# achiever04/face-recognition-platform

Hardware: AMD Instinct MI355X
Metric: faces/sec (detect+embed+match) on 1080p @ 100k gallery (higher is better)
Workload: dtype f16; 1 GPU; 32x1080x1920 BGR frames per GPU per step resident in HBM, host results out every step, 2 batches in flight per GPU (one handle = one stream each, used round-robin), forced K=10 faces/frame, 100000-identity fp16 gallery, FRPDet detector fp16 + ArcFace IResNet-100 fp16 (synthetic seeded weights); batch_frames=32, faces_per_frame=10, gallery=100000, streams=1, lanes=2, lane_warmup_steps=20

## Files before the change

face-recognition-platform_amd/csrc/decode_nms.hip:

```cpp
#include <hip/hip_runtime.h>
#include <stdint.h>
#include "frp_internal.h"

namespace frp {

#define NMS_CAP 1024
#define NT 1024

__device__ __forceinline__ unsigned sortable16(unsigned short h) {
    if ((h & 0x7fffu) > 0x7c00u) return 0u;
    return (h & 0x8000u) ? (unsigned)(unsigned short)(~h) : (unsigned)(h | 0x8000u);
}
__device__ __forceinline__ bool is_candidate(_Float16 lg, float lt) {
    return lt == -INFINITY ? true : (float)lg >= lt;
}

struct FrameView {
    const _Float16 *h0, *h1, *h2;
    int w0, w1, w2;
    int e0, e1;
};

__device__ __forceinline__ const _Float16* anchor_ptr(const FrameView& fv, int idx, int& level, int& x, int& y) {
    level = idx < fv.e0 ? 0 : (idx < fv.e1 ? 1 : 2);
    const int li = idx - (level == 0 ? 0 : (level == 1 ? fv.e0 : fv.e1));
    const int wl = level == 0 ? fv.w0 : (level == 1 ? fv.w1 : fv.w2);
    const _Float16* base = level == 0 ? fv.h0 : (level == 1 ? fv.h1 : fv.h2);
    const int pos = li >> 1, a = li & 1;
    y = pos / wl;
    x = pos - y * wl;
    return base + (long)pos * 32 + a * 15;
}

__device__ __forceinline__ FrameView frame_view(const DecodeParams& p, int b, int& A) {
    FrameView fv;
    fv.h0 = p.head[0] + (long)b * p.hl[0] * p.wl[0] * 32;
    fv.h1 = p.head[1] + (long)b * p.hl[1] * p.wl[1] * 32;
    fv.h2 = p.head[2] + (long)b * p.hl[2] * p.wl[2] * 32;
    fv.w0 = p.wl[0]; fv.w1 = p.wl[1]; fv.w2 = p.wl[2];
    fv.e0 = p.hl[0] * p.wl[0] * 2;
    fv.e1 = fv.e0 + p.hl[1] * p.wl[1] * 2;
    A = fv.e1 + p.hl[2] * p.wl[2] * 2;
    return fv;
}

__global__ __launch_bounds__(256) void gather_logits_kernel(DecodeParams p) {
    int A;
    const FrameView fv = frame_view(p, blockIdx.y, A);
    const int i = blockIdx.x * 256 + threadIdx.x;
    if (i >= A) return;
    int lv, x, y;
    p.logits[(long)blockIdx.y * A + i] = anchor_ptr(fv, i, lv, x, y)[0];
}

__global__ __launch_bounds__(NT) void decode_nms_kernel(DecodeParams p) {
    __shared__ unsigned long long keys[NMS_CAP];
    __shared__ int hist[4096];
    __shared__ float bx1[NMS_CAP], by1[NMS_CAP], bx2[NMS_CAP], by2[NMS_CAP], barea[NMS_CAP];
    __shared__ unsigned char supp[NMS_CAP];
    __shared__ int s_cnt, s_digit, s_need, s_keepn;
    __shared__ int s_keep[FRP_MAX_FACES_CAP];
    __shared__ int wsum[NT / 64];

    const int b = blockIdx.x;
    const int tid = threadIdx.x;
    int A;
    const FrameView fv = frame_view(p, b, A);
    const float lt = p.logit_thresh;

    if (tid == 0) { s_cnt = 0; s_keepn = 0; }
    __syncthreads();
    const _Float16* dense = p.logits + (long)b * A;
    int local = 0;
    for (int i = tid; i < A; i += NT) local += is_candidate(dense[i], lt) ? 1 : 0;
#pragma unroll
    for (int o = 32; o > 0; o >>= 1) local += __shfl_xor(local, o);
    if ((tid & 63) == 0) atomicAdd(&s_cnt, local);
    __syncthreads();
    const int total = s_cnt;
    __syncthreads();

    unsigned long long T = 0ull;
    if (total > NMS_CAP) {
        unsigned long long prefix = 0ull;
        int need = NMS_CAP;
        for (int pass = 0; pass < 3; ++pass) {
            const int shift = 24 - 12 * pass;
            for (int i = tid; i < 4096; i += NT) hist[i] = 0;
            __syncthreads();
            for (int i = tid; i < A; i += NT) {
                const _Float16 lg = dense[i];
                if (is_candidate(lg, lt)) {
                    const unsigned long long k = ((unsigned long long)sortable16(__builtin_bit_cast(unsigned short, lg)) << 20) |
                                                 (unsigned long long)(0xFFFFF - i);
                    if (pass == 0 || (k >> (shift + 12)) == prefix) atomicAdd(&hist[(int)((k >> shift) & 0xFFF)], 1);
                }
            }
            __syncthreads();
            const int b0 = tid * 4;
            const int h0 = hist[b0], h1 = hist[b0 + 1], h2 = hist[b0 + 2], h3 = hist[b0 + 3];
            const int mine = h0 + h1 + h2 + h3;
            int v = mine;
#pragma unroll
            for (int o = 1; o < 64; o <<= 1) {
                const int n = __shfl_down(v, o);
                if ((tid & 63) + o < 64) v += n;
            }
            if ((tid & 63) == 0) wsum[tid >> 6] = v;
            __syncthreads();
            int above_waves = 0;
            for (int w = (tid >> 6) + 1; w < NT / 64; ++w) above_waves += wsum[w];
            const int suffix_incl = v + above_waves;
            const int above = suffix_incl - mine;
            int c = above;
            if (c < need && need <= c + h3) { s_digit = b0 + 3; s_need = need - c; }
            c += h3;
            if (c < need && need <= c + h2) { s_digit = b0 + 2; s_need = need - c; }
            c += h2;
            if (c < need && need <= c + h1) { s_digit = b0 + 1; s_need = need - c; }
            c += h1;
            if (c < need && need <= c + h0) { s_digit = b0; s_need = need - c; }
            __syncthreads();
            prefix = (prefix << 12) | (unsigned long long)s_digit;
            need = s_need;
            __syncthreads();
        }
        T = prefix;
    }

    if (tid == 0) s_cnt = 0;
    for (int i = tid; i < NMS_CAP; i += NT) { keys[i] = 0ull; supp[i] = 0; }
    __syncthreads();
    for (int i = tid; i < A; i += NT) {
        const _Float16 lg = dense[i];
        if (is_candidate(lg, lt)) {
            const unsigned long long k = ((unsigned long long)sortable16(__builtin_bit_cast(unsigned short, lg)) << 20) |
                                         (unsigned long long)(0xFFFFF - i);
            if (k >= T) {
                const int s = atomicAdd(&s_cnt, 1);
                if (s < NMS_CAP) keys[s] = k | (1ull << 40);
            }
        }
    }
    __syncthreads();
    const int n = s_cnt < NMS_CAP ? s_cnt : NMS_CAP;

    for (int k2 = 2; k2 <= NMS_CAP; k2 <<= 1) {
        for (int j = k2 >> 1; j > 0; j >>= 1) {
            const int i = tid;
            const int ixj = i ^ j;
            if (ixj > i) {
                const unsigned long long a = keys[i], c = keys[ixj];
                const bool desc = (i & k2) == 0;
                if (desc ? (a < c) : (a > c)) { keys[i] = c; keys[ixj] = a; }
            }
            __syncthreads();
        }
    }

    if (tid < n) {
        const int idx = 0xFFFFF - (int)(keys[tid] & 0xFFFFF);
        int lv, x, y;
        const _Float16* q = anchor_ptr(fv, idx, lv, x, y);
        const float s = (float)(8 << lv);
        const float cx = (float)(x * (8 << lv)), cy = (float)(y * (8 << lv));
        const float x1 = cx - (float)q[1] * s, y1 = cy - (float)q[2] * s;
        const float x2 = cx + (float)q[3] * s, y2 = cy + (float)q[4] * s;
        bx1[tid] = x1; by1[tid] = y1; bx2[tid] = x2; by2[tid] = y2;
        barea[tid] = (x2 - x1 + 1.0f) * (y2 - y1 + 1.0f);
    }
    __syncthreads();

    const int K = p.max_faces;
    for (int i = 0; i < n; ++i) {
        if (supp[i]) continue;
        if (tid == 0) s_keep[s_keepn] = i;
        const int kept = s_keepn + 1;
// ... 59 lines not shown
        const uint8_t* p00 = src + (((long)b * H + y0) * W + x0) * 3;
        const uint8_t* p01 = src + (((long)b * H + y0) * W + x1) * 3;
        const uint8_t* p10 = src + (((long)b * H + y1) * W + x0) * 3;
        const uint8_t* p11 = src + (((long)b * H + y1) * W + x1) * 3;
        uint8_t* o = dst + i * 3;
#pragma unroll
        for (int c = 0; c < 3; ++c) {
            const float top = (float)p00[c] * (1.0f - fx) + (float)p01[c] * fx;
            const float bot = (float)p10[c] * (1.0f - fx) + (float)p11[c] * fx;
            const float v = top * (1.0f - fy) + bot * fy;
            o[c] = (uint8_t)fminf(fmaxf(floorf(v + 0.5f), 0.0f), 255.0f);
        }
    }
}

hipError_t launch_resize_u8(const uint8_t* src, int B, int H, int W, uint8_t* dst, int Hs, int Ws, hipStream_t stream) {
    if (!src || !dst || B <= 0 || H <= 0 || W <= 0 || Hs <= 0 || Ws <= 0) return hipErrorInvalidValue;
    const long total = (long)B * Hs * Ws;
    const int grid = (int)((total + 255) / 256 < 16384 ? (total + 255) / 256 : 16384);
    hipLaunchKernelGGL(resize_u8_kernel, dim3(grid), dim3(256), 0, stream, src, B, H, W, dst, Hs, Ws,
                       (float)H / (float)Hs, (float)W / (float)Ws);
    return hipGetLastError();
}

hipError_t launch_decode_nms(const DecodeParams& p, hipStream_t stream) {
    if (p.B <= 0 || p.max_faces <= 0 || p.max_faces > FRP_MAX_FACES_CAP) return hipErrorInvalidValue;
    long A = 0;
    for (int l = 0; l < 3; ++l) {
        if (!p.head[l] || p.hl[l] <= 0 || p.wl[l] <= 0) return hipErrorInvalidValue;
        A += (long)p.hl[l] * p.wl[l] * 2;
    }
    if (A > 0xFFFFF) return hipErrorInvalidValue;
    if (!p.boxes || !p.kps || !p.scores || !p.counts || !p.logits) return hipErrorInvalidValue;
    hipLaunchKernelGGL(gather_logits_kernel, dim3((unsigned)((A + 255) / 256), p.B), dim3(256), 0, stream, p);
    hipError_t e = hipGetLastError();
    if (e != hipSuccess) return e;
    hipLaunchKernelGGL(decode_nms_kernel, dim3(p.B), dim3(NT), 0, stream, p);
    return hipGetLastError();
}

}
```

face-recognition-platform_amd/csrc/frp_api.cpp:

```cpp
#include <hip/hip_runtime.h>

#include <algorithm>
#include <cmath>
#include <cstdio>
#include <cstdlib>
#include <cstring>
#include <mutex>
#include <string>
#include <vector>

#include "frp.h"
#include "frp_blob.h"
#include "frp_internal.h"
#include "frp_handle.h"

using namespace frp;

#define FRP_WINO_MIN_FACES 128
Switches frp::read_switches() {
    auto set = [](const char* n) { return getenv(n) ? 1 : 0; };
    const char *sm = getenv("FRP_SMALL_M"), *wm = getenv("FRP_WINO_MIN_FACES");
    Switches s{};
    s.small_m = !sm ? 0 : (sm[0] == '0' ? -1 : 1);
    s.wino_min_faces = wm ? atoi(wm) : FRP_WINO_MIN_FACES;
    s.s2 = set("FRP_S2"); s.host_count = set("FRP_HOST_COUNT"); s.match_v1 = set("FRP_MATCH_V1");
    s.no_fused_stem12 = set("FRP_NO_FUSED_STEM12"); s.no_fused_stem = set("FRP_NO_FUSED_STEM");
    s.no_emb_stem = set("FRP_NO_EMB_STEM"); s.no_stem_fuse = set("FRP_NO_STEM_FUSE");
    s.no_wino = set("FRP_NO_WINO"); s.no_kconcat = set("FRP_NO_KCONCAT");
    s.no_block_fuse = set("FRP_NO_BLOCK_FUSE"); s.block_fuse_all = set("FRP_BLOCK_FUSE_ALL");
    return s;
}

const ProcessSwitches& frp::process_switches() {
    static const ProcessSwitches s = [] {
        const char* jh = getenv("FRP_JPEG_DEVICE_HUFFMAN");
        const char* js = getenv("FRP_JPEG_SELFSYNC");
        return ProcessSwitches{getenv("FRP_NO_GRAPH") != nullptr, getenv("FRP_C64_ALL") != nullptr, !jh ? 0 : (jh[0] == '0' ? -1 : 1), js && js[0] != '0'};
    }();
    return s;
}

namespace {

float logit_threshold(float t) {
    if (!(t > 0.f)) return -INFINITY;
    if (t >= 1.f) return INFINITY;
    return (float)std::log((double)t / (1.0 - (double)t));
}

bool det_size_ok(int Hs, int Ws) { return Hs > 0 && Ws > 0 && Hs <= 16384 && Ws <= 16384; }

int select_det_source(frp_handle* h, int Hs, int Ws) {
    if (h->rB <= 0) return fail(h, FRP_ERR_INVALID, "no resident frames (call frp_upload_frames)");
    if (!det_size_ok(Hs, Ws)) return fail(h, FRP_ERR_INVALID, "bad detector size");
    if (Hs == h->rH && Ws == h->rW) {
        h->det_scaled = false;
    } else {
        FRPCHK(ensure(h, h->scaled, (size_t)h->rB * Hs * Ws * 3));
        hipError_t e = launch_resize_u8((const uint8_t*)h->frames.p, h->rB, h->rH, h->rW, (uint8_t*)h->scaled.p, Hs, Ws, h->stream);
        if (e != hipSuccess) return fail(h, FRP_ERR_HIP, std::string("resize: ") + hipGetErrorString(e));
        h->det_scaled = true;
    }
    h->dH = Hs; h->dW = Ws;
    h->canvas_h = round_up(Hs, 32);
    h->canvas_w = round_up(Ws, 32);
    return FRP_OK;
}

int ensure_results(frp_handle* h, int B, int K) {
    const size_t s = (size_t)B * K;
    FRPCHK(ensure(h, h->boxes, s * 4 * 4));
    FRPCHK(ensure(h, h->kps, s * 10 * 4));
    FRPCHK(ensure(h, h->scores, s * 4));
    FRPCHK(ensure(h, h->anchor, s * 4));
    FRPCHK(ensure(h, h->counts, (size_t)B * 4));
    FRPCHK(ensure(h, h->face_slot, s * 4));
    FRPCHK(ensure(h, h->nfaces, 16));
    return FRP_OK;
}

struct DetOut {
    float *boxes, *kps, *scores;
    int32_t* counts;
};

int run_decode(frp_handle* h, const void* const head[3], const int dims[3][2], int B, int K, float det_thresh, float nms_iou, uint32_t flags,
               const DetOut* out = nullptr) {
    DecodeParams dp{};
    size_t anchors = 0;
    for (int l = 0; l < 3; ++l) {
        dp.head[l] = (const _Float16*)head[l];
        dp.hl[l] = dims[l][0];
        dp.wl[l] = dims[l][1];
        anchors += (size_t)dp.hl[l] * dp.wl[l] * 2;
    }
    dp.B = B;
    dp.max_faces = K;
    const bool forced = flags & FRP_FLAG_FORCED_K;
    dp.logit_thresh = forced ? -INFINITY : logit_threshold(det_thresh);
    dp.nms_iou = forced ? 2.0f : nms_iou;
    if (out) {
        dp.boxes = out->boxes; dp.kps = out->kps; dp.scores = out->scores; dp.counts = out->counts;
    } else {
        dp.boxes = (float*)h->boxes.p; dp.kps = (float*)h->kps.p; dp.scores = (float*)h->scores.p;
        dp.anchor = (int32_t*)h->anchor.p; dp.counts = (int32_t*)h->counts.p;
    }
    FRPCHK(ensure(h, h->dense_logits, (size_t)B * anchors * 2));
    dp.logits = (_Float16*)h->dense_logits.p;
    const hipError_t e = launch_decode_nms(dp, h->stream);
    if (e != hipSuccess) return fail(h, FRP_ERR_HIP, std::string("decode_nms: ") + hipGetErrorString(e));
    return FRP_OK;
}

int compact_faces(frp_handle* h, int B, int K) {
    hipError_t e = launch_compact_faces((const int32_t*)h->counts.p, B, K, (int32_t*)h->face_slot.p, (int32_t*)h->nfaces.p, h->stream);
    if (e != hipSuccess) return fail(h, FRP_ERR_HIP, std::string("compact_faces: ") + hipGetErrorString(e));
    return FRP_OK;
}

StemParams stem_params(const frp_handle* h, uint32_t flags) {
    StemParams sp{};
    sp.frames = h->det_scaled ? (const uint8_t*)h->scaled.p : (const uint8_t*)h->frames.p;
    sp.B = h->rB; sp.H = h->dH; sp.W = h->dW;
    sp.row_stride = (long)h->dW * 3; sp.frame_stride = (long)h->dH * h->dW * 3;
    sp.Hc = h->canvas_h; sp.Wc = h->canvas_w; sp.Ho = sp.Hc / 2; sp.Wo = sp.Wc / 2;
    sp.rgb_in = (flags & FRP_FLAG_RGB) ? 1 : 0;
    return sp;
}

bool det_wino(const frp_handle* h) {
    return (long)h->rB * (h->canvas_h / 8) * (h->canvas_w / 8) >= 2L * 240 * (h->n_cu > 0 ? h->n_cu : 256);
}

int run_detect(frp_handle* h, const Switches& sw, int K, float det_thresh, float nms_iou, uint32_t flags, const DetOut* out = nullptr) {
    if (!h->have_weights) return fail(h, FRP_ERR_NO_WEIGHTS, "no weights loaded");
    if (h->rB <= 0) return fail(h, FRP_ERR_INVALID, "no resident frames (call frp_upload_frames)");
    if (K <= 0 || K > FRP_MAX_FACES_CAP) return fail(h, FRP_ERR_INVALID, "max_faces out of range");
    const int B = h->rB, Hc = h->canvas_h, Wc = h->canvas_w;
    const bool fused = h->det.det_stem && !sw.no_fused_stem;
    FRPCHK(plan_net(h, h->det, B, Hc, Wc, fused));
    if (!out) FRPCHK(ensure_results(h, B, K));
    const StemParams sp = stem_params(h, flags);
    if (!fused) {
        hipError_t e = launch_preprocess(sp.frames, B, sp.H, sp.W, sp.row_stride, sp.frame_stride, (_Float16*)h->det.bufs[h->det.in_buf].p, Hc, Wc,
                                         sp.rgb_in, h->stream);
        if (e != hipSuccess) return fail(h, FRP_ERR_HIP, std::string("preprocess: ") + hipGetErrorString(e));
    }
    rec(h, EV_PRE);
    FRPCHK(run_net(h, sw, h->det, B, Hc, Wc, &h->ctr.det_conv_flops, &h->ctr.det_conv_launches, fused ? &sp : nullptr, nullptr, det_wino(h)));
    rec(h, EV_DET);
    const void* head[3];
    int dims[3][2];
    for (int l = 0; l < 3; ++l) {
        const int bi = (int)h->hdr.det_head_buf[l];
        head[l] = h->det.bufs[bi].p;
        dims[l][0] = h->det.dims[bi].h;
        dims[l][1] = h->det.dims[bi].w;
        if (h->det.dims[bi].c != 32) return fail(h, FRP_ERR_BLOB, "detector head must have 32 channels");
    }
    FRPCHK(run_decode(h, head, dims, B, K, det_thresh, nms_iou, flags, out));
    if (!out && !(flags & FRP_FLAG_TRACK)) FRPCHK(compact_faces(h, B, K));
    rec(h, EV_DEC);
    return FRP_OK;
}

int run_embed(frp_handle* h, const Switches& sw, int n, const int32_t* n_dev = nullptr, int family_count = -1) {
    if (n <= 0) return FRP_OK;
    if (family_count < 0) family_count = n;
    FcSplitK fc;
    FRPCHK(run_net(h, sw, h->emb, n, FRP_CHIP, FRP_CHIP, &h->ctr.emb_conv_flops, &h->ctr.emb_conv_launches, nullptr, n_dev,
                   family_count >= sw.wino_min_faces, &fc));
    rec(h, EV_EMB);
    FRPCHK(stage_queries(h, n));
    hipError_t e = launch_l2norm((float*)h->emb.bufs[h->hdr.emb_out_buf].p, (_Float16*)h->m.q16.p, n, FRP_EMB_DIM, h->stream,
                                 fc.ksplit != 0 && fc.ksplit != 1 ? (const float*)h->splitk_ws.p : nullptr, fc.ksplit, fc.bias, n_dev, fc.ktot,
                                 h->n_cu);
    if (e != hipSuccess) return fail(h, FRP_ERR_HIP, std::string("l2norm: ") + hipGetErrorString(e));
    rec(h, EV_L2);
    return FRP_OK;
}

int run_align(frp_handle* h, int K, int n, const int32_t* n_dev, uint32_t flags, void* chips) {
    AlignParams ap{};
    ap.frames = (const uint8_t*)h->frames.p;
    ap.B = h->rB; ap.H = h->rH; ap.W = h->rW;
    ap.row_stride = (long)h->rW * 3;
    ap.frame_stride = (long)h->rH * h->rW * 3;
    ap.kps = (const float*)h->kps.p;
    if (K > 0) {
        ap.counts = (const int32_t*)h->counts.p;
        ap.face_slot = (const int32_t*)h->face_slot.p;
    }
    ap.max_faces = K > 0 ? K : n;
// ... 278 lines not shown
    h->cfg.max_batch = 32; h->cfg.max_faces = 10; h->cfg.max_h = 1080; h->cfg.max_w = 1920; h->cfg.profile = 0;
    if (cfg) {
        if (cfg->struct_size != (int32_t)sizeof(frp_config)) { delete h; return FRP_ERR_INVALID; }
        if (cfg->max_batch > 0) h->cfg.max_batch = cfg->max_batch;
        if (cfg->max_faces > 0) h->cfg.max_faces = std::min<int>(cfg->max_faces, FRP_MAX_FACES_CAP);
        if (cfg->max_h > 0) h->cfg.max_h = cfg->max_h;
        if (cfg->max_w > 0) h->cfg.max_w = cfg->max_w;
        h->cfg.profile = cfg->profile ? 1 : 0;
    }
    bool ok = hipSetDevice(device) == hipSuccess && hipStreamCreateWithFlags(&h->stream, hipStreamNonBlocking) == hipSuccess;
    for (int i = 0; ok && i < EV_COUNT; ++i) ok = hipEventCreate(&h->ev[i]) == hipSuccess;
    ok = ok && hipHostMalloc((void**)&h->h_nfaces, 64, hipHostMallocDefault) == hipSuccess;
    if (ok) {
        hipDeviceProp_t prop;
        if (hipGetDeviceProperties(&prop, device) == hipSuccess && prop.multiProcessorCount > 0) h->n_cu = prop.multiProcessorCount;
    }
    ok = ok && init_ingest(h);
    if (!ok) { frp_destroy(h); return FRP_ERR_HIP; }
    h->ctr.struct_size = sizeof(frp_counters);
    *out = h;
    return FRP_OK;
}

void frp_destroy(frp_handle* h) {
    if (!h) return;
    (void)hipSetDevice(h->device);
    if (h->stream) (void)hipStreamSynchronize(h->stream);
    if (h->in.copy_stream) (void)hipStreamSynchronize(h->in.copy_stream);
    dist_shutdown(h);
    drop_graphs(h);
    for (DevBuf& b : h->det.bufs) release(b);
    for (DevBuf& b : h->emb.bufs) release(b);
    DevBuf* all[] = {&h->wdata, &h->frames, &h->boxes, &h->kps, &h->scores, &h->counts, &h->anchor, &h->face_slot, &h->nfaces,
                     &h->pyr_boxes, &h->pyr_kps, &h->pyr_scores, &h->pyr_counts, &h->m.q16, &h->m.part_cos, &h->m.part_idx, &h->m.best_cos, &h->m.best_idx, &h->m.hit_cnt, &h->m.hit_idx, &h->m.hit_cos, &h->m.q_groups, &h->m.frame_groups_dev, &h->g_groups_dev, &h->scratch, &h->splitk_ws, &h->dense_logits, &h->scaled, &h->gallery,
                     &h->g_reserved, &h->gx, &h->gx_q, &h->gx_out, &h->det_hashes, &h->quality_in, &h->quality_out,
                     &h->jenc_in, &h->jenc_coef, &h->jenc_work, &h->jenc_bits, &h->jenc_out, &h->enh_in, &h->enh_out};
    for (DevBuf* b : all) release(*b);
    for (int i = 0; i < EV_COUNT; ++i) if (h->ev[i]) (void)hipEventDestroy(h->ev[i]);
    if (h->m.frame_groups_ev) (void)hipEventDestroy(h->m.frame_groups_ev);
    release_tracks(h);
    if (h->h_nfaces) (void)hipHostFree(h->h_nfaces);
    if (h->pin_stage) (void)hipHostFree(h->pin_stage);
    release_ingest(h);
    if (h->stream) (void)hipStreamDestroy(h->stream);
    delete h;
}

const char* frp_last_error(const frp_handle* h) { return h ? h->err.c_str() : "null handle"; }

int frp_load_weights(frp_handle* h, const void* blob, size_t bytes) {
    if (!h) return FRP_ERR_INVALID;
    Guard g(h);
    h->have_weights = false;
    ++h->alloc_epoch;
    if (!blob || bytes < sizeof(frp_blob_header)) return fail(h, FRP_ERR_BLOB, "blob too small");
    frp_blob_header hd;
    memcpy(&hd, blob, sizeof(hd));
    if (memcmp(hd.magic, FRP_BLOB_MAGIC, 8) != 0 || hd.version != FRP_BLOB_VERSION || hd.header_bytes != sizeof(frp_blob_header))
        return fail(h, FRP_ERR_BLOB, "bad magic/version");
    if (hd.data_offset > bytes || hd.data_bytes > bytes - hd.data_offset) return fail(h, FRP_ERR_BLOB, "data section out of range");
    if (hd.emb_dim != FRP_EMB_DIM || hd.emb_size != FRP_CHIP || hd.det_in_ch != 8 || hd.emb_in_ch != 8 || hd.det_num_anchors != 2)
        return fail(h, FRP_ERR_BLOB, "unsupported network geometry");
    std::vector<unsigned char> image;
    FRPCHK(load_program(h, hd, (const unsigned char*)blob, bytes, read_switches(), image));
    FRPCHK(ensure(h, h->wdata, image.size()));
    HIPCHK(h, hipMemcpyAsync(h->wdata.p, image.data(), image.size(), hipMemcpyHostToDevice, h->stream));
    HIPCHK(h, hipStreamSynchronize(h->stream));
// ... 183 lines not shown
    const TensorDims d = h->det.dims[op.out_buf];
    if (th) *th = d.h;
    if (tw) *tw = d.w;
    if (tc) *tc = d.c;
    const int64_t need = (int64_t)B * d.h * d.w * d.c * 2;
    if (!out_f16) { HIPCHK(h, hipStreamSynchronize(h->stream)); return FRP_OK; }
    if (out_bytes < need) return fail(h, FRP_ERR_INVALID, "tensor buffer too small");
    return copy_out(h, out_f16, h->det.bufs[op.out_buf].p, (size_t)need);
}

int frp_decode_heads(frp_handle* h, const void* head8, const void* head16, const void* head32, int32_t B, int32_t canvas_h,
                     int32_t canvas_w, int32_t max_faces, float det_thresh, float nms_iou, uint32_t flags, float* boxes,
                     float* kps, float* scores, int32_t* counts, int32_t* anchor_idx) {
    if (!h) return FRP_ERR_INVALID;
    Guard g(h);
    if (!head8 || !head16 || !head32 || B <= 0 || B > 1024 || canvas_h <= 0 || canvas_w <= 0 || (canvas_h & 31) || (canvas_w & 31) ||
        max_faces <= 0 || max_faces > FRP_MAX_FACES_CAP)
        return fail(h, FRP_ERR_INVALID, "bad decode arguments");
    const void* src[3] = {head8, head16, head32};
    ScopedBuf tmp[3];
    const int rc = [&]() -> int {
        const void* head[3];
        int dims[3][2];
        for (int l = 0; l < 3; ++l) {
            dims[l][0] = canvas_h / (8 << l);
            dims[l][1] = canvas_w / (8 << l);
            const size_t bytes = (size_t)B * dims[l][0] * dims[l][1] * 32 * 2;
            FRPCHK(ensure(h, tmp[l], bytes));
            if (hipMemcpyAsync(tmp[l]->p, src[l], bytes, hipMemcpyHostToDevice, h->stream) != hipSuccess)
                return fail(h, FRP_ERR_HIP, "head upload failed");
            head[l] = tmp[l]->p;
        }
        FRPCHK(ensure_results(h, B, max_faces));
        FRPCHK(run_decode(h, head, dims, B, max_faces, det_thresh, nms_iou, flags));
        return copy_detections_out(h, B, max_faces, boxes, kps, scores, counts, anchor_idx);
    }();
    if (rc != FRP_OK) (void)hipStreamSynchronize(h->stream);
    return rc;
}

static int align_common(frp_handle* h, const uint8_t* bgr, int H, int W, int64_t row_stride, const float* kps, int M, uint32_t flags,
                        bool to_embedder) {
    if (to_embedder && !h->have_weights) return fail(h, FRP_ERR_NO_WEIGHTS, "no weights loaded");
    if (!kps || M <= 0 || M > 65536) return fail(h, FRP_ERR_INVALID, "bad landmark arguments");
    FRPCHK(upload_frames(h, bgr, 1, H, W, row_stride));
    if (to_embedder) FRPCHK(plan_net(h, h->emb, M, FRP_CHIP, FRP_CHIP));
    else FRPCHK(ensure(h, h->scratch, (size_t)M * FRP_CHIP_PIX * 16));
    FRPCHK(ensure(h, h->kps, (size_t)M * 40));
    HIPCHK(h, hipMemcpyAsync(h->kps.p, kps, (size_t)M * 40, hipMemcpyHostToDevice, h->stream));
    return run_align(h, 0, M, nullptr, flags, to_embedder ? h->emb.bufs[h->emb.in_buf].p : h->scratch.p);
}

int frp_align(frp_handle* h, const uint8_t* bgr, int32_t H, int32_t W, int64_t row_stride, const float* kps, int32_t M,
              uint32_t flags, void* chips_f16) {
    if (!h) return FRP_ERR_INVALID;
    Guard g(h);
    if (!chips_f16) return fail(h, FRP_ERR_INVALID, "null output");
    FRPCHK(align_common(h, bgr, H, W, row_stride, kps, M, flags, false));
    return copy_out(h, chips_f16, h->scratch.p, (size_t)M * FRP_CHIP_PIX * 8 * 2);
}

int frp_debug_align_resident(frp_handle* h, const float* kps, const int32_t* counts, int32_t max_faces, uint32_t flags,
                             int32_t device_count, void* chips_f16, int64_t out_bytes) {
    if (!h) return FRP_ERR_INVALID;
    Guard g(h);
    if (h->rB <= 0) return fail(h, FRP_ERR_INVALID, "no resident frames (call frp_upload_frames)");
    const int B = h->rB, K = max_faces;
// ... 62 lines not shown
```

face-recognition-platform_amd/csrc/frp_handle.h:

```cpp
#pragma once
#include <hip/hip_runtime.h>

#include <algorithm>
#include <mutex>
#include <string>
#include <utility>
#include <vector>

#include "frp.h"
#include "frp_blob.h"
#include "frp_internal.h"
#include "net_program.h"

enum { EV_START = 0, EV_H2D, EV_PRE, EV_DET, EV_DEC, EV_ALIGN, EV_EMB, EV_L2, EV_MATCH, EV_D2H, EV_COUNT };

struct Ingest {
    frp::DevBuf frames_next;
    int nB = 0, nH = 0, nW = 0;
    bool next_valid = false;
    hipStream_t copy_stream = nullptr;
    hipEvent_t ev_next_ready = nullptr, ev_next_free = nullptr;
    std::vector<void*> pinned;
    void* jpeg_pin[2] = {nullptr, nullptr};
    size_t jpeg_pin_cap[2] = {0, 0};
// ... 53 lines not shown
    bool tracked = false, track_matched = false;
    int pend_cap = 0;
    double pend_flops = 0.0, pend_f8flops = 0.0;
};

struct frp_handle {
    int device = 0;
    hipStream_t stream = nullptr;
    std::mutex mu;
    std::string err;
    frp_config cfg{};
    bool have_weights = false;
    frp_blob_header hdr{};
    frp::DevBuf wdata;
    frp::Net det, emb;
    frp::DevBuf frames;
    int rB = 0, rH = 0, rW = 0;
    int n_cu = 256;
    Ingest in;
    frp::DevBuf scaled;
    int dH = 0, dW = 0;
    bool det_scaled = false;
    int canvas_h = 0, canvas_w = 0;
    int det_op_limit = -1;
    std::vector<frp::NetGraph> graphs;
    std::vector<std::string> graph_seen, graph_bad;
    uint64_t alloc_epoch = 1;
    int64_t graph_replays = 0;
    void* comm = nullptr;
    int dist_rank = 0, dist_world = 0;
    frp::DevBuf det_hashes;
    bool det_hash_on = false;
    frp::DevBuf boxes, kps, scores, counts, anchor, face_slot, nfaces, scratch, splitk_ws, dense_logits;
    frp::DevBuf pyr_boxes, pyr_kps, pyr_scores, pyr_counts;
    Matcher m;
    Pass pass;
    Tracks trk;
    bool ev_pending = false;
    frp::DevBuf quality_in, quality_out;
    frp::DevBuf jenc_in, jenc_coef, jenc_work, jenc_bits, jenc_out;
    frp::DevBuf enh_in, enh_out;
    int32_t* h_nfaces = nullptr;
    unsigned char* pin_stage = nullptr;
    size_t pin_cap = 0;
    frp::DevBuf gallery;
    int64_t g_rows = 0;
    frp::DevBuf g_reserved;
    bool g_exact = false;
    frp::DevBuf gx, gx_q, gx_out;
    std::vector<uint32_t> g_groups;
    frp::DevBuf g_groups_dev;
    bool g_groups_dev_ok = false;
    hipEvent_t ev[EV_COUNT]{};
    frp_counters ctr{};
};

namespace frp {

inline int fail(frp_handle* h, int code, const std::string& msg) {
    if (h) h->err = msg;
    return code;
}

#define HIPCHK(h, expr)                                                                              \
    do {                                                                                             \
        hipError_t _e = (expr);                                                                      \
// ... 84 lines not shown
```

face-recognition-platform_amd/csrc/frp_internal.h:

```cpp
#pragma once
#include <hip/hip_runtime.h>
#include <stdint.h>
#include <type_traits>

#define FRP_ACT_NONE 0
#define FRP_ACT_RELU 1
#define FRP_ACT_PRELU 2
#define FRP_FLAG_BORDER_BIAS 1
#define FRP_FLAG_OUT_F32 2
#define FRP_FLAG_RES_UP2 4
#define FRP_FLAG_FLATTEN 8
#define FRP_FLAG_F8 32
#define FRP_FLAG_OUT_FP8 64
#define FRP_CHIP_PIX (112 * 112)
#ifndef FRP_MAX_FACES_CAP
#define FRP_MAX_FACES_CAP 128
#endif

#include "jpeg_host.h"
#include "jpeg_selfsync.h"

namespace frp {

struct Switches {
    int small_m;
    int s2;
    int no_fused_stem12;
    int no_fused_stem;
    int no_emb_stem;
    int no_stem_fuse;
    int wino_min_faces;
    int host_count;
    int match_v1;
    int no_wino;
    int no_kconcat;
    int no_block_fuse;
    int block_fuse_all;
};
static_assert(std::has_unique_object_representations_v<Switches>, "run_net keys captured graphs by the bytes of a Switches");
Switches read_switches();

struct ProcessSwitches {
    bool no_graph;
    bool c64_all;
    int jpeg_device_huffman;
    bool jpeg_selfsync;
};
const ProcessSwitches& process_switches();

struct ConvParams {
    const _Float16* x;
    const _Float16* w;
    const float* bias;
    const float* slope;
    const _Float16* res;
    void* out;
    void* out2;
    const _Float16* x2;
    int Cin2;
    const float* wscale;
    float in_scale;
    float out_scale;
    int N, H, W, Cin, Cout, KS, stride;
    int act, flags;
    int Hr, Wr;
    int ksplit;
    const _Float16* wino_w;
    const int32_t* n_dev;
    int n_cu;
    unsigned long long* stamps;
// ... 135 lines not shown
    const _Float16* w;
    const float* bias;
    _Float16* out;
};
hipError_t launch_stem_u8(const StemParams& p, hipStream_t stream);

struct Stem12Params {
    const uint8_t* frames;
    int B, H, W;
    long row_stride, frame_stride;
    int Hc, Wc;
    int Ho1, Wo1;
    int Ho2, Wo2;
    int rgb_in;
    const _Float16* w1;
    const float* bias1;
    const _Float16* w2;
    const float* bias2;
    _Float16* out;
};
hipError_t launch_stem12_u8(const Stem12Params& p, hipStream_t stream);

struct EmbStemParams {
    const _Float16* x;
    int M, H, W;
    const _Float16* w;
    const float* bias;
    const float* slope;
    _Float16* out;
    const int32_t* n_dev;
};
hipError_t launch_emb_stem(const EmbStemParams& p, hipStream_t stream);

struct DecodeParams {
    const _Float16* head[3];
    int hl[3], wl[3];
    int B, max_faces;
    float logit_thresh, nms_iou;
    float* boxes;
    float* kps;
    float* scores;
    int32_t* anchor;
    int32_t* counts;
    _Float16* logits;
};
hipError_t launch_decode_nms(const DecodeParams& p, hipStream_t stream);

#define FRP_PYRAMID_MAX_SCALES 4
#define FRP_PYRAMID_MAX_CAND 512
struct PyramidMergeParams {
    const float* boxes;
    const float* kps;
    const float* scores;
    const int32_t* counts;
    int S, B, P, max_faces;
    int frame_h, frame_w;
    int det_h[FRP_PYRAMID_MAX_SCALES], det_w[FRP_PYRAMID_MAX_SCALES];
    float nms_iou;
    float* out_boxes;
    float* out_kps;
    float* out_scores;
    int32_t* out_anchor;
    int32_t* out_counts;
    float rx[FRP_PYRAMID_MAX_SCALES], ry[FRP_PYRAMID_MAX_SCALES];
};
hipError_t launch_pyramid_merge(PyramidMergeParams p, hipStream_t stream);

struct JpegParams {
    const int16_t* coef;
    const uint16_t* qtab;
    uint8_t* planes;
    uint8_t* frames;
    int B, W, H, components;
    int bx[3], by[3];
    int blocks_per_image;
    long plane_off[3], plane_img;
    int hs, vs;
// ... 272 lines not shown
```

Before: 28650 faces/s.

## Split decode top-K selection into grid-wide histogram and candidate-append kernels

Replaces the per-frame single-block radix select, which scanned every anchor logit up to four times, with two grid-parallel kernels. The first fuses the logit gather with a 12-bit score histogram. The second finds the threshold digit and appends sure candidates plus a boundary-digit list to global buffers. The NMS kernel then only refines the boundary list with a two-pass select. It adds per-frame selection state that must be zeroed between calls, global atomics, and a fallback to the old dense path when the boundary bucket overflows.

New measurement: 28730 faces/s, median of 6. Within noise of the previous version (+0.3%).

```diff
diff --git a/face-recognition-platform_amd/csrc/decode_nms.hip b/face-recognition-platform_amd/csrc/decode_nms.hip
--- a/face-recognition-platform_amd/csrc/decode_nms.hip
+++ b/face-recognition-platform_amd/csrc/decode_nms.hip
@@ -53,9 +53,211 @@
     p.logits[(long)blockIdx.y * A + i] = anchor_ptr(fv, i, lv, x, y)[0];
 }
 
+#define BCAP FRP_DECODE_BCAP
+#define SEL_NT 256
+#define SEL_CHUNK 4096
+static_assert(NMS_CAP == FRP_DECODE_CAP && BCAP == 4096 && SEL_CHUNK == 16 * SEL_NT, "list sizes and chunking the kernels are written for");
+static_assert(sizeof(DecodeSel) % 16 == 0 && offsetof(DecodeSel, hist) == 0, "16-byte loads and stores of a frame's histogram");
+
+__device__ __forceinline__ unsigned long long anchor_key(_Float16 lg, int i) {
+    return ((unsigned long long)sortable16(__builtin_bit_cast(unsigned short, lg)) << 20) | (unsigned long long)(0xFFFFF - i);
+}
+
+__global__ __launch_bounds__(SEL_NT) void gather_hist_kernel(DecodeParams p) {
+    __shared__ unsigned lh[4096];
+    int A;
+    const FrameView fv = frame_view(p, blockIdx.y, A);
+    const int tid = threadIdx.x;
+#pragma unroll
+    for (int k = 0; k < 16; ++k) lh[k * SEL_NT + tid] = 0u;
+    __syncthreads();
+    const int base = blockIdx.x * SEL_CHUNK + tid;
+    const float lt = p.logit_thresh;
+    _Float16 lg[16];
+#pragma unroll
+    for (int k = 0; k < 16; ++k) {
+        const int i = base + k * SEL_NT;
+        int lv, x, y;
+        lg[k] = i < A ? anchor_ptr(fv, i, lv, x, y)[0] : (_Float16)0;
+    }
+    _Float16* dense = p.logits + (long)blockIdx.y * A;
+#pragma unroll
+    for (int k = 0; k < 16; ++k) {
+        const int i = base + k * SEL_NT;
+        if (i < A) {
+            dense[i] = lg[k];
+            if (is_candidate(lg[k], lt)) atomicAdd(&lh[sortable16(__builtin_bit_cast(unsigned short, lg[k])) >> 4], 1u);
+        }
+    }
+    __syncthreads();
+    unsigned* gh = p.sel[blockIdx.y].hist;
+#pragma unroll
+    for (int k = 0; k < 16; ++k) {
+        const unsigned c = lh[k * SEL_NT + tid];
+        if (c) atomicAdd(&gh[k * SEL_NT + tid], c);
+    }
+}
+
+__global__ __launch_bounds__(SEL_NT) void append_candidates_kernel(DecodeParams p) {
+    __shared__ int wsum[SEL_NT / 64];
+    __shared__ int s_digit, s_need, s_dense;
+    __shared__ unsigned s_base[2];
+    const int b = blockIdx.y, tid = threadIdx.x;
+    DecodeSel* fs = p.sel + b;
+
+    unsigned hb[16];
+    {
+        const uint4* h4 = reinterpret_cast<const uint4*>(fs->hist) + tid * 4;
+#pragma unroll
+        for (int k = 0; k < 4; ++k) {
+            const uint4 v = h4[k];
+            hb[4 * k] = v.x; hb[4 * k + 1] = v.y; hb[4 * k + 2] = v.z; hb[4 * k + 3] = v.w;
+        }
+    }
+    int mine = 0;
+#pragma unroll
+    for (int k = 0; k < 16; ++k) mine += (int)hb[k];
+    int v = mine;
+#pragma unroll
+    for (int o = 1; o < 64; o <<= 1) {
+        const int n = __shfl_down(v, o);
+        if ((tid & 63) + o < 64) v += n;
+    }
+    if ((tid & 63) == 0) wsum[tid >> 6] = v;
+    if (tid == 0) { s_digit = -1; s_need = 0; s_dense = 0; }
+    __syncthreads();
+    int above = v - mine, total = 0;
+#pragma unroll
+    for (int w = 0; w < SEL_NT / 64; ++w) {
+        total += wsum[w];
+        if (w > (tid >> 6)) above += wsum[w];
+    }
+    if (total > NMS_CAP && above < NMS_CAP && NMS_CAP <= above + mine) {
+        int c = above;
+#pragma unroll
+        for (int k = 15; k >= 0; --k) {
+            if (c < NMS_CAP && NMS_CAP <= c + (int)hb[k]) { s_digit = tid * 16 + k; s_need = NMS_CAP - c; s_dense = hb[k] > BCAP ? 1 : 0; }
+            c += (int)hb[k];
+        }
+    }
+    __syncthreads();
+    const int d = s_digit;
+    if (blockIdx.x == 0 && tid == 0) { fs->total = total; fs->digit = d; fs->need = s_need; fs->dense = s_dense; }
+    if (s_dense) return;
+
+    int A;
+    (void)frame_view(p, b, A);
+    const long lo = (long)b * A, hi = lo + A;
+    const long v0 = (lo + 7) & ~7L;
+    const long v1 = (hi & ~7L) > v0 ? (hi & ~7L) : v0;
+    const float lt = p.logit_thresh;
+    uint4 vec[2];
+    long at[3];
+    _Float16 sc = (_Float16)0;
+#pragma unroll
+    for (int k = 0; k < 2; ++k) {
+        const long e = v0 + ((long)blockIdx.x * (SEL_CHUNK / 8) + k * SEL_NT + tid) * 8;
+        at[k] = e < v1 ? e : -1;
+        vec[k] = at[k] >= 0 ? *reinterpret_cast<const uint4*>(p.logits + e) : make_uint4(0, 0, 0, 0);
+    }
+    at[2] = -1;
+    if (blockIdx.x == 0 && tid < 7 && lo + tid < (v0 < hi ? v0 : hi)) at[2] = lo + tid;
+    if (blockIdx.x == 0 && tid >= 8 && tid < 15 && v1 + (tid - 8) < hi) at[2] = v1 + (tid - 8);
+    if (at[2] >= 0) sc = p.logits[at[2]];
+
+    auto cls = [&](_Float16 lg) -> int {
+        if (!is_candidate(lg, lt)) return 0;
+        const int dg = (int)(sortable16(__builtin_bit_cast(unsigned short, lg)) >> 4);
+        return dg > d ? 1 : (dg == d ? 2 : 0);
+    };
+    auto half_of = [](const uint4& q, int j) -> _Float16 {
+        const unsigned w = j < 2 ? q.x : (j < 4 ? q.y : (j < 6 ? q.z : q.w));
+        return __builtin_bit_cast(_Float16, (unsigned short)((j & 1) ? (w >> 16) : (w & 0xFFFFu)));
+    };
+    int cnt = 0;
+#pragma unroll
+    for (int k = 0; k < 2; ++k)
+        if (at[k] >= 0) {
+#pragma unroll
+            for (int j = 0; j < 8; ++j) {
+                const int c = cls(half_of(vec[k], j));
+                cnt += c == 1 ? 1 : (c == 2 ? 0x10000 : 0);
+            }
+        }
+    if (at[2] >= 0) { const int c = cls(sc); cnt += c == 1 ? 1 : (c == 2 ? 0x10000 : 0); }
+
+    int incl = cnt;
+#pragma unroll
+    for (int o = 1; o < 64; o <<= 1) {
+        const int n = __shfl_up(incl, o);
+        if ((tid & 63) >= o) incl += n;
+    }
+    __syncthreads();
+    if ((tid & 63) == 63) wsum[tid >> 6] = incl;
+    __syncthreads();
+    int before = incl - cnt, wg_total = 0;
+#pragma unroll
+    for (int w = 0; w < SEL_NT / 64; ++w) {
+        wg_total += wsum[w];
+        if (w < (tid >> 6)) before += wsum[w];
+    }
+    if (tid == 0) {
+        s_base[0] = (wg_total & 0xFFFF) ? atomicAdd(&fs->n_cand, (unsigned)(wg_total & 0xFFFF)) : 0u;
+        s_base[1] = (wg_total >> 16) ? atomicAdd(&fs->n_bnd, (unsigned)(wg_total >> 16)) : 0u;
+    }
+    __syncthreads();
+    unsigned sc_c = s_base[0] + (unsigned)(before & 0xFFFF), sc_b = s_base[1] + (unsigned)(before >> 16);
+    unsigned long long* cand = p.cand + (long)b * NMS_CAP;
+    unsigned* bnd = p.bnd + (long)b * BCAP;
+    auto put = [&](_Float16 lg, long e) {
+        const int c = cls(lg);
+        if (c == 0) return;
+        const unsigned long long key = anchor_key(lg, (int)(e - lo));
+        if (c == 1 && sc_c < NMS_CAP) cand[sc_c] = key;
+        if (c == 2 && sc_b < BCAP) bnd[sc_b] = (unsigned)(key & 0xFFFFFFull);
+        sc_c += c == 1 ? 1u : 0u;
+        sc_b += c == 2 ? 1u : 0u;
+    };
+#pragma unroll
+    for (int k = 0; k < 2; ++k)
+        if (at[k] >= 0) {
+#pragma unroll
+            for (int j = 0; j < 8; ++j) put(half_of(vec[k], j), at[k] + j);
+        }
+    if (at[2] >= 0) put(sc, at[2]);
+}
+
+__device__ __forceinline__ void pick_digit(const int* hist, int* wsum, int need, int tid, int* s_digit, int* s_need) {
+    const int b0 = tid * 4;
+    const int h0 = hist[b0], h1 = hist[b0 + 1], h2 = hist[b0 + 2], h3 = hist[b0 + 3];
+    const int mine = h0 + h1 + h2 + h3;
+    int v = mine;
+#pragma unroll
+    for (int o = 1; o < 64; o <<= 1) {
+        const int n = __shfl_down(v, o);
+        if ((tid & 63) + o < 64) v += n;
+    }
+    if ((tid & 63) == 0) wsum[tid >> 6] = v;
+    __syncthreads();
+    int above_waves = 0;
+    for (int w = (tid >> 6) + 1; w < NT / 64; ++w) above_waves += wsum[w];
+    const int suffix_incl = v + above_waves;
+    const int above = suffix_incl - mine;
+    int c = above;
+    if (c < need && need <= c + h3) { *s_digit = b0 + 3; *s_need = need - c; }
+    c += h3;
+    if (c < need && need <= c + h2) { *s_digit = b0 + 2; *s_need = need - c; }
+    c += h2;
+    if (c < need && need <= c + h1) { *s_digit = b0 + 1; *s_need = need - c; }
+    c += h1;
+    if (c < need && need <= c + h0) { *s_digit = b0; *s_need = need - c; }
+    __syncthreads();
+}
+
 __global__ __launch_bounds__(NT) void decode_nms_kernel(DecodeParams p) {
     __shared__ unsigned long long keys[NMS_CAP];
     __shared__ int hist[4096];
+    __shared__ unsigned blist[BCAP];
     __shared__ float bx1[NMS_CAP], by1[NMS_CAP], bx2[NMS_CAP], by2[NMS_CAP], barea[NMS_CAP];
     __shared__ unsigned char supp[NMS_CAP];
     __shared__ int s_cnt, s_digit, s_need, s_keepn;
@@ -68,81 +270,104 @@
     const FrameView fv = frame_view(p, b, A);
     const float lt = p.logit_thresh;
 
+    DecodeSel* fs = p.dense_route ? nullptr : p.sel + b;
+    const bool lists = fs && !fs->dense;
     if (tid == 0) { s_cnt = 0; s_keepn = 0; }
-    __syncthreads();
-    const _Float16* dense = p.logits + (long)b * A;
-    int local = 0;
-    for (int i = tid; i < A; i += NT) local += is_candidate(dense[i], lt) ? 1 : 0;
-#pragma unroll
-    for (int o = 32; o > 0; o >>= 1) local += __shfl_xor(local, o);
-    if ((tid & 63) == 0) atomicAdd(&s_cnt, local);
-    __syncthreads();
-    const int total = s_cnt;
-    __syncthreads();
-
-    unsigned long long T = 0ull;
-    if (total > NMS_CAP) {
-        unsigned long long prefix = 0ull;
-        int need = NMS_CAP;
-        for (int pass = 0; pass < 3; ++pass) {
-            const int shift = 24 - 12 * pass;
-            for (int i = tid; i < 4096; i += NT) hist[i] = 0;
+    for (int i = tid; i < NMS_CAP; i += NT) { keys[i] = 0ull; supp[i] = 0; }
+    __syncthreads();
+
+    if (lists) {
+        const int d = fs->digit;
+        const int n_c = (int)(fs->n_cand < NMS_CAP ? fs->n_cand : NMS_CAP);
+        const unsigned long long* cand = p.cand + (long)b * NMS_CAP;
+        for (int i = tid; i < n_c; i += NT) keys[i] = cand[i] | (1ull << 40);
+        if (tid == 0) s_cnt = n_c;
+        if (d >= 0) {
+            const int n_b = (int)(fs->n_bnd < BCAP ? fs->n_bnd : BCAP);
+            int need = fs->need < n_b ? fs->need : n_b;
+            const unsigned* bnd = p.bnd + (long)b * BCAP;
+            for (int i = tid; i < n_b; i += NT) blist[i] = bnd[i];
+            unsigned T24 = 0u;
+            if (need < n_b) {
+                unsigned prefix = 0u;
+                for (int pass = 0; pass < 2; ++pass) {
+                    const int shift = 12 - 12 * pass;
+                    for (int i = tid; i < 4096; i += NT) hist[i] = 0;
+                    __syncthreads();
+                    for (int i = tid; i < n_b; i += NT) {
+                        const unsigned k = blist[i];
+                        if (pass == 0 || (k >> 12) == prefix) atomicAdd(&hist[(int)((k >> shift) & 0xFFF)], 1);
+                    }
+                    __syncthreads();
+                    pick_digit(hist, wsum, need, tid, &s_digit, &s_need);
+                    prefix = (prefix << 12) | (unsigned)s_digit;
+                    need = s_need;
+                    __syncthreads();
+                }
+                T24 = prefix;
+            }
             __syncthreads();
-            for (int i = tid; i < A; i += NT) {
-                const _Float16 lg = dense[i];
-                if (is_candidate(lg, lt)) {
-                    const unsigned long long k = ((unsigned long long)sortable16(__builtin_bit_cast(unsigned short, lg)) << 20) |
-                                                 (unsigned long long)(0xFFFFF - i);
-                    if (pass == 0 || (k >> (shift + 12)) == prefix) atomicAdd(&hist[(int)((k >> shift) & 0xFFF)], 1);
+            for (int i = tid; i < n_b; i += NT) {
+                const unsigned k = blist[i];
+                if (k >= T24) {
+                    const int s = atomicAdd(&s_cnt, 1);
+                    if (s < NMS_CAP) keys[s] = ((unsigned long long)d << 24) | k | (1ull << 40);
                 }
             }
-            __syncthreads();
-            const int b0 = tid * 4;
-            const int h0 = hist[b0], h1 = hist[b0 + 1], h2 = hist[b0 + 2], h3 = hist[b0 + 3];
-            const int mine = h0 + h1 + h2 + h3;
-            int v = mine;
-#pragma unroll
-            for (int o = 1; o < 64; o <<= 1) {
-                const int n = __shfl_down(v, o);
-                if ((tid & 63) + o < 64) v += n;
-            }
-            if ((tid & 63) == 0) wsum[tid >> 6] = v;
-            __syncthreads();
-            int above_waves = 0;
-            for (int w = (tid >> 6) + 1; w < NT / 64; ++w) above_waves += wsum[w];
-            const int suffix_incl = v + above_waves;
-            const int above = suffix_incl - mine;
-            int c = above;
-            if (c < need && need <= c + h3) { s_digit = b0 + 3; s_need = need - c; }
-            c += h3;
-            if (c < need && need <= c + h2) { s_digit = b0 + 2; s_need = need - c; }
-            c += h2;
-            if (c < need && need <= c + h1) { s_digit = b0 + 1; s_need = need - c; }
-            c += h1;
-            if (c < need && need <= c + h0) { s_digit = b0; s_need = need - c; }
-            __syncthreads();
-            prefix = (prefix << 12) | (unsigned long long)s_digit;
-            need = s_need;
-            __syncthreads();
-        }
-        T = prefix;
-    }
-
-    if (tid == 0) s_cnt = 0;
-    for (int i = tid; i < NMS_CAP; i += NT) { keys[i] = 0ull; supp[i] = 0; }
-    __syncthreads();
-    for (int i = tid; i < A; i += NT) {
-        const _Float16 lg = dense[i];
-        if (is_candidate(lg, lt)) {
-            const unsigned long long k = ((unsigned long long)sortable16(__builtin_bit_cast(unsigned short, lg)) << 20) |
-                                         (unsigned long long)(0xFFFFF - i);
-            if (k >= T) {
-                const int s = atomicAdd(&s_cnt, 1);
-                if (s < NMS_CAP) keys[s] = k | (1ull << 40);
-            }
-        }
-    }
-    __syncthreads();
+        }
+    } else {
+        const _Float16* dense = p.logits + (long)b * A;
+        int local = 0;
+        for (int i = tid; i < A; i += NT) local += is_candidate(dense[i], lt) ? 1 : 0;
+#pragma unroll
+        for (int o = 32; o > 0; o >>= 1) local += __shfl_xor(local, o);
+        if ((tid & 63) == 0) atomicAdd(&s_cnt, local);
+        __syncthreads();
+        const int total = s_cnt;
+        __syncthreads();
+
+        unsigned long long T = 0ull;
+        if (total > NMS_CAP) {
+            unsigned long long prefix = 0ull;
+            int need = NMS_CAP;
+            for (int pass = 0; pass < 3; ++pass) {
+                const int shift = 24 - 12 * pass;
+                for (int i = tid; i < 4096; i += NT) hist[i] = 0;
+                __syncthreads();
+                for (int i = tid; i < A; i += NT) {
+                    const _Float16 lg = dense[i];
+                    if (is_candidate(lg, lt)) {
+                        const unsigned long long k = anchor_key(lg, i);
+                        if (pass == 0 || (k >> (shift + 12)) == prefix) atomicAdd(&hist[(int)((k >> shift) & 0xFFF)], 1);
+                    }
+                }
+                __syncthreads();
+                pick_digit(hist, wsum, need, tid, &s_digit, &s_need);
+                prefix = (prefix << 12) | (unsigned long long)s_digit;
+                need = s_need;
+                __syncthreads();
+            }
+            T = prefix;
+        }
+
+        if (tid == 0) s_cnt = 0;
+        __syncthreads();
+        for (int i = tid; i < A; i += NT) {
+            const _Float16 lg = dense[i];
+            if (is_candidate(lg, lt)) {
+                const unsigned long long k = anchor_key(lg, i);
+                if (k >= T) {
+                    const int s = atomicAdd(&s_cnt, 1);
+                    if (s < NMS_CAP) keys[s] = k | (1ull << 40);
+                }
+            }
+        }
+    }
+    __syncthreads();
+    if (fs) {
+        reinterpret_cast<uint4*>(fs->hist)[tid] = make_uint4(0, 0, 0, 0);
+        if (tid == 0) { fs->n_cand = 0u; fs->n_bnd = 0u; }
+    }
     const int n = s_cnt < NMS_CAP ? s_cnt : NMS_CAP;
 
     for (int k2 = 2; k2 <= NMS_CAP; k2 <<= 1) {
@@ -268,11 +493,27 @@
     }
     if (A > 0xFFFFF) return hipErrorInvalidValue;
     if (!p.boxes || !p.kps || !p.scores || !p.counts || !p.logits) return hipErrorInvalidValue;
-    hipLaunchKernelGGL(gather_logits_kernel, dim3((unsigned)((A + 255) / 256), p.B), dim3(256), 0, stream, p);
+    if (p.dense_route) {
+        hipLaunchKernelGGL(gather_logits_kernel, dim3((unsigned)((A + 255) / 256), p.B), dim3(256), 0, stream, p);
+        hipError_t e = hipGetLastError();
+        if (e != hipSuccess) return e;
+        hipLaunchKernelGGL(decode_nms_kernel, dim3(p.B), dim3(NT), 0, stream, p);
+        return hipGetLastError();
+    }
+    if (!p.sel || !p.cand || !p.bnd || ((uintptr_t)p.logits & 15)) return hipErrorInvalidValue;
+    const dim3 chunks((unsigned)((A + SEL_CHUNK - 1) / SEL_CHUNK), p.B);
+    hipLaunchKernelGGL(gather_hist_kernel, chunks, dim3(SEL_NT), 0, stream, p);
     hipError_t e = hipGetLastError();
-    if (e != hipSuccess) return e;
-    hipLaunchKernelGGL(decode_nms_kernel, dim3(p.B), dim3(NT), 0, stream, p);
-    return hipGetLastError();
-}
-
-}
+    if (e == hipSuccess) {
+        hipLaunchKernelGGL(append_candidates_kernel, chunks, dim3(SEL_NT), 0, stream, p);
+        e = hipGetLastError();
+    }
+    if (e == hipSuccess) {
+        hipLaunchKernelGGL(decode_nms_kernel, dim3(p.B), dim3(NT), 0, stream, p);
+        e = hipGetLastError();
+    }
+    if (e != hipSuccess) (void)hipMemsetAsync(p.sel, 0, (size_t)p.B * sizeof(DecodeSel), stream);
+    return e;
+}
+
+}
diff --git a/face-recognition-platform_amd/csrc/frp_api.cpp b/face-recognition-platform_amd/csrc/frp_api.cpp
--- a/face-recognition-platform_amd/csrc/frp_api.cpp
+++ b/face-recognition-platform_amd/csrc/frp_api.cpp
@@ -28,6 +28,7 @@
     s.no_emb_stem = set("FRP_NO_EMB_STEM"); s.no_stem_fuse = set("FRP_NO_STEM_FUSE");
     s.no_wino = set("FRP_NO_WINO"); s.no_kconcat = set("FRP_NO_KCONCAT");
     s.no_block_fuse = set("FRP_NO_BLOCK_FUSE"); s.block_fuse_all = set("FRP_BLOCK_FUSE_ALL");
+    s.decode_dense = set("FRP_DECODE_DENSE");
     return s;
 }
 
@@ -84,8 +85,8 @@
     int32_t* counts;
 };
 
-int run_decode(frp_handle* h, const void* const head[3], const int dims[3][2], int B, int K, float det_thresh, float nms_iou, uint32_t flags,
-               const DetOut* out = nullptr) {
+int run_decode(frp_handle* h, const Switches& sw, const void* const head[3], const int dims[3][2], int B, int K, float det_thresh, float nms_iou,
+               uint32_t flags, const DetOut* out = nullptr) {
     DecodeParams dp{};
     size_t anchors = 0;
     for (int l = 0; l < 3; ++l) {
@@ -107,6 +108,17 @@
     }
     FRPCHK(ensure(h, h->dense_logits, (size_t)B * anchors * 2));
     dp.logits = (_Float16*)h->dense_logits.p;
+    dp.dense_route = sw.decode_dense;
+    if (!dp.dense_route) {
+        const size_t cap0 = h->decode_sel.cap;
+        FRPCHK(ensure(h, h->decode_sel, (size_t)B * sizeof(DecodeSel)));
+        if (h->decode_sel.cap != cap0) HIPCHK(h, hipMemsetAsync(h->decode_sel.p, 0, h->decode_sel.cap, h->stream));
+        FRPCHK(ensure(h, h->decode_cand, (size_t)B * FRP_DECODE_CAP * sizeof(unsigned long long)));
+        FRPCHK(ensure(h, h->decode_bnd, (size_t)B * FRP_DECODE_BCAP * sizeof(unsigned)));
+        dp.sel = (DecodeSel*)h->decode_sel.p;
+        dp.cand = (unsigned long long*)h->decode_cand.p;
+        dp.bnd = (unsigned*)h->decode_bnd.p;
+    }
     const hipError_t e = launch_decode_nms(dp, h->stream);
     if (e != hipSuccess) return fail(h, FRP_ERR_HIP, std::string("decode_nms: ") + hipGetErrorString(e));
     return FRP_OK;
@@ -158,7 +170,7 @@
         dims[l][1] = h->det.dims[bi].w;
         if (h->det.dims[bi].c != 32) return fail(h, FRP_ERR_BLOB, "detector head must have 32 channels");
     }
-    FRPCHK(run_decode(h, head, dims, B, K, det_thresh, nms_iou, flags, out));
+    FRPCHK(run_decode(h, sw, head, dims, B, K, det_thresh, nms_iou, flags, out));
     if (!out && !(flags & FRP_FLAG_TRACK)) FRPCHK(compact_faces(h, B, K));
     rec(h, EV_DEC);
     return FRP_OK;
@@ -503,7 +515,7 @@
     for (DevBuf& b : h->det.bufs) release(b);
     for (DevBuf& b : h->emb.bufs) release(b);
     DevBuf* all[] = {&h->wdata, &h->frames, &h->boxes, &h->kps, &h->scores, &h->counts, &h->anchor, &h->face_slot, &h->nfaces,
-                     &h->pyr_boxes, &h->pyr_kps, &h->pyr_scores, &h->pyr_counts, &h->m.q16, &h->m.part_cos, &h->m.part_idx, &h->m.best_cos, &h->m.best_idx, &h->m.hit_cnt, &h->m.hit_idx, &h->m.hit_cos, &h->m.q_groups, &h->m.frame_groups_dev, &h->g_groups_dev, &h->scratch, &h->splitk_ws, &h->dense_logits, &h->scaled, &h->gallery,
+                     &h->pyr_boxes, &h->pyr_kps, &h->pyr_scores, &h->pyr_counts, &h->m.q16, &h->m.part_cos, &h->m.part_idx, &h->m.best_cos, &h->m.best_idx, &h->m.hit_cnt, &h->m.hit_idx, &h->m.hit_cos, &h->m.q_groups, &h->m.frame_groups_dev, &h->g_groups_dev, &h->scratch, &h->splitk_ws, &h->dense_logits, &h->decode_sel, &h->decode_cand, &h->decode_bnd, &h->scaled, &h->gallery,
                      &h->g_reserved, &h->gx, &h->gx_q, &h->gx_out, &h->det_hashes, &h->quality_in, &h->quality_out,
                      &h->jenc_in, &h->jenc_coef, &h->jenc_work, &h->jenc_bits, &h->jenc_out, &h->enh_in, &h->enh_out};
     for (DevBuf* b : all) release(*b);
@@ -753,7 +765,7 @@
             head[l] = tmp[l]->p;
         }
         FRPCHK(ensure_results(h, B, max_faces));
-        FRPCHK(run_decode(h, head, dims, B, max_faces, det_thresh, nms_iou, flags));
+        FRPCHK(run_decode(h, read_switches(), head, dims, B, max_faces, det_thresh, nms_iou, flags));
         return copy_detections_out(h, B, max_faces, boxes, kps, scores, counts, anchor_idx);
     }();
     if (rc != FRP_OK) (void)hipStreamSynchronize(h->stream);
diff --git a/face-recognition-platform_amd/csrc/frp_handle.h b/face-recognition-platform_amd/csrc/frp_handle.h
--- a/face-recognition-platform_amd/csrc/frp_handle.h
+++ b/face-recognition-platform_amd/csrc/frp_handle.h
@@ -109,6 +109,7 @@
     frp::DevBuf det_hashes;
     bool det_hash_on = false;
     frp::DevBuf boxes, kps, scores, counts, anchor, face_slot, nfaces, scratch, splitk_ws, dense_logits;
+    frp::DevBuf decode_sel, decode_cand, decode_bnd;
     frp::DevBuf pyr_boxes, pyr_kps, pyr_scores, pyr_counts;
     Matcher m;
     Pass pass;
diff --git a/face-recognition-platform_amd/csrc/frp_internal.h b/face-recognition-platform_amd/csrc/frp_internal.h
--- a/face-recognition-platform_amd/csrc/frp_internal.h
+++ b/face-recognition-platform_amd/csrc/frp_internal.h
@@ -36,6 +36,7 @@
     int no_kconcat;
     int no_block_fuse;
     int block_fuse_all;
+    int decode_dense;
 };
 static_assert(std::has_unique_object_representations_v<Switches>, "run_net keys captured graphs by the bytes of a Switches");
 Switches read_switches();
@@ -237,6 +238,15 @@
 };
 hipError_t launch_emb_stem(const EmbStemParams& p, hipStream_t stream);
 
+#define FRP_DECODE_CAP 1024
+#define FRP_DECODE_BCAP 4096
+struct DecodeSel {
+    unsigned hist[4096];
+    int total, digit, need;
+    int dense;
+    unsigned n_cand, n_bnd;
+    unsigned pad[2];
+};
 struct DecodeParams {
     const _Float16* head[3];
     int hl[3], wl[3];
@@ -248,6 +258,10 @@
     int32_t* anchor;
     int32_t* counts;
     _Float16* logits;
+    DecodeSel* sel;
+    unsigned long long* cand;
+    unsigned* bnd;
+    int dense_route;
 };
 hipError_t launch_decode_nms(const DecodeParams& p, hipStream_t stream);
 
```
